# jac99/Egonn

Measured on AMD Instinct MI355X. Metric: LiDAR scans/sec (descriptor extraction), 50k-pt clouds @ 0.1m voxel, higher is better.
Workload: dtype f32

## Files before the change

egonn_amd/_lib.py:

```python
from __future__ import annotations

import ctypes as C
import os
from typing import List, Optional, Sequence

import numpy as np
import torch

_HERE = os.path.dirname(os.path.abspath(__file__))
LIB_PATH = os.path.join(_HERE, "lib", "libegonn_hip.so")

QUANT_CARTESIAN, QUANT_POLAR = 0, 1
FLAG_DISABLE_GLOBAL, FLAG_DISABLE_LOCAL, FLAG_IGNORE_KP_REGRESSOR, FLAG_BF16 = 1, 2, 4, 8
FLAG_POOL_SPOC, FLAG_POOL_MAC = 16, 32
MINKFPN_SPLIT_TOPDOWN = 1
MINKFPN_BLOCKS = {'BasicBlock': 0, 'ECABasicBlock': 1}
MINKFPN_POOLING = {None: 0, 'GeM': 1, 'MAC': 2, 'SPoC': 3}

_P = C.c_void_p
_SIGS = [
    ("egonn_ctx_create", C.c_int, [C.POINTER(_P), C.c_int, C.c_int]),
    ("egonn_ctx_destroy", None, [_P]),
    ("egonn_last_error", C.c_char_p, []),
    ("egonn_debug_set_naive_conv", C.c_int, [_P, C.c_int]),
    ("egonn_debug_set_ksplit", C.c_int, [_P, C.c_int, C.c_int, C.c_int, C.c_int, C.c_int]),
    ("egonn_debug_set_resident", C.c_int, [_P, C.c_int, C.c_int]),
    ("egonn_debug_keep_level_features", C.c_int, [_P, C.c_int]),
    ("egonn_debug_set_trace", C.c_int, [_P]),
    ("egonn_prepare_maps", C.c_int, [_P, C.c_int, _P]),
    ("egonn_debug_rowgroup_tables", C.c_int, [_P, C.c_int, C.c_int, _P, _P, C.c_int64, C.POINTER(C.c_int64), _P]),
    ("egonn_debug_rowgroup_perm", C.c_int, [_P, C.c_int, C.c_int, _P, C.c_int64, C.POINTER(C.c_int64), _P]),
    ("egonn_debug_radix_sort_scratch_bytes", C.c_int64, [C.c_int64, C.c_int]),
    ("egonn_debug_radix_sort", C.c_int, [_P, _P, _P, _P, C.c_int64, C.c_int, _P, _P, C.c_int, C.c_int, C.c_int,
                                         C.POINTER(C.c_int32), _P, C.c_int64, _P]),
    ("egonn_debug_dense_group3", C.c_int, [_P, _P, _P, _P, _P, _P, _P]),
    ("egonn_debug_global_tail_scratch_bytes", C.c_int64, [C.c_int64]),
    ("egonn_debug_global_tail", C.c_int, [_P, _P, C.c_int, C.c_int64, _P, _P, _P, _P, _P, _P, C.c_int, C.c_int, _P, _P, _P, C.c_int64, _P]),
    ("egonn_voxelize", C.c_int, [_P, _P, C.POINTER(C.c_int64), C.c_int, C.c_int, C.POINTER(C.c_float), _P]),
    ("egonn_ctx_reserve", C.c_int, [_P, C.c_int64, C.c_int, C.POINTER(C.c_int64)]),
    ("egonn_voxelize_device", C.c_int, [_P, _P, C.c_int64, _P, C.c_int, C.c_int, C.POINTER(C.c_float), _P]),
    ("egonn_plan_status", C.c_int, [_P, _P]),
    ("egonn_ctx_set_exact_fp32", C.c_int, [_P, C.c_int]),
    ("egonn_ctx_set_operand_autoscale", C.c_int, [_P, C.c_int]),
    ("egonn_level_capacity", C.c_int, [_P, C.c_int, C.POINTER(C.c_int64)]),
    ("egonn_graph_begin", C.c_int, [_P]),
    ("egonn_graph_end", C.c_int, [_P, C.POINTER(_P)]),
# ... 277 lines not shown
                       "gx", "gy", "gz", "block", "lds", "kparts")


def debug_sconv_choice(kind: int, level: int, cin: int, cout: int, cap_groups: int, *, code: int = 0, bf16: int = 0, gated: int = 0,
                       split_io: int = 0, residual: int = 0, split_max_level: int = 5, autoscale: int = 0, resident_mask: int = -1,
                       max_workgroups: int = 0, kparts: int = -1, kw: int = -1, col_parts: int = -1) -> dict:
    arg = (C.c_int32 * 16)(int(code), kind, level, cin, cout, int(bf16), int(gated), split_io, int(residual), split_max_level,
                           int(autoscale), resident_mask, max_workgroups, kparts, kw, col_parts)
    out = (C.c_int32 * 20)()
    check(load().egonn_debug_sconv_choice(arg, int(cap_groups), out))
    d = dict(zip(SCONV_CHOICE_FIELDS, out))
    d["route"], d["kernel"] = SCONV_ROUTES[d["route"]], SCONV_ROUTES[d["kernel"]]
    return d


DENSE_ROUTES = ("none", "stream", "lds", "small", "tile", "plain")


def debug_dense_route(rows: int, cin: int, cout: int, form: int = -1, gate_scans: int = 0):
    out = (C.c_int32 * 5)()
    check(load().egonn_debug_dense_route(int(rows), int(cin), int(cout), int(form), int(gate_scans), out))
    return (DENSE_ROUTES[out[0]],) + tuple(out[1:])


def debug_radix_sort(keys_in, vals_in, keys_out, vals_out, n: int, nbits: int, n_dev=None, seg_offsets=None, idx_bits: int = 0,
                     either_pair: bool = False, scratch_buf=None, scratch_bytes: Optional[int] = None) -> int:
    lib = load()
    B = 0 if seg_offsets is None else seg_offsets.numel() - 1
    need = lib.egonn_debug_radix_sort_scratch_bytes(int(n), B)
    if scratch_buf is None:
# ... 180 lines not shown
        ng, _ = self.map_groups(map_kind, level_out)
        K = 27 if map_kind == 0 else 8
        gm = torch.empty(ng, dtype=torch.int32, device=self.device)
        sn = torch.empty((ng, K, 16), dtype=torch.int32, device=self.device) if with_rows else None
        n = C.c_int64()
        self._call(self.lib.egonn_debug_rowgroup_tables, self.h, map_kind, level_out, gm.data_ptr(),
                   sn.data_ptr() if with_rows else None, ng, C.byref(n))
        return gm, sn

    def rowgroup_perm(self, map_kind: int, level_out: int):
        ng, _ = self.map_groups(map_kind, level_out)
        pm = torch.empty((ng, 16), dtype=torch.int32, device=self.device)
        n = C.c_int64()
        self._call(self.lib.egonn_debug_rowgroup_perm, self.h, map_kind, level_out, pm.data_ptr(), ng, C.byref(n))
        return pm

    def set_naive_conv(self, on):
        check(self.lib.egonn_debug_set_naive_conv(self.h, int(on)))

    def keep_level_features(self, on: bool):
        check(self.lib.egonn_debug_keep_level_features(self.h, int(bool(on))))

    def set_exact_fp32(self, on: bool):
        check(self.lib.egonn_ctx_set_exact_fp32(self.h, int(bool(on))))

    def set_operand_autoscale(self, on: bool):
        check(self.lib.egonn_ctx_set_operand_autoscale(self.h, int(bool(on))))

    def set_ksplit(self, map_class: int, level: int, kparts: int = -1, kw: int = -1, col_parts: int = -1):
        check(self.lib.egonn_debug_set_ksplit(self.h, int(map_class), int(level), int(kparts), int(kw), int(col_parts)))
# ... 390 lines not shown
```

egonn_amd/csrc/common.h:

```cpp
#pragma once
#include <hip/hip_runtime.h>
#include <atomic>
#include <stdint.h>
#include <stdio.h>
#include <string.h>
#include <string>
#include <vector>

#define EGONN_MAX_LEVELS 10
#define EGONN_NUM_LEVELS 8
#define EGONN_MAX_BATCH 4096

#define API extern "C" __attribute__((visibility("default")))

namespace egonn {

void set_error(const char* fmt, ...);
#define EGONN_OK 0
#define EGONN_ERR_INVALID 1
#define EGONN_ERR_HIP 2
#define EGONN_ERR_RANGE 3
#define EGONN_ERR_STATE 4
#define EGONN_ERR_CAPACITY 5
#define EGONN_ERR_FP16_RANGE 6
// ... 139 lines not shown
struct Plan {
  bool valid = false;
  bool built_reserved = false;
  bool exact = false;
  int64_t cap_points = 0;
  int64_t* scan_off = nullptr;
  int batch = 0;
  int coord_bits = 16;
  int64_t n_input = 0;
  Level lv[EGONN_MAX_LEVELS];
  int64_t cap[EGONN_MAX_LEVELS] = {};
  int32_t* perm0 = nullptr;
  int32_t* g0 = nullptr;
  uint64_t* t2m = nullptr;
  int32_t* t2s = nullptr;
  std::vector<int32_t> boff_host[EGONN_NUM_LEVELS];
};

enum ProfKind { PK_CONV0 = 0, PK_K3 = 1, PK_K2S2 = 2, PK_TCONV = 3, PK_OTHER = 4 };
struct ProfRec {
  char name[64];
  int kind, level, K, cin, cout;
  int es;
  hipEvent_t e0, e1;
};
struct Profiler {
  int mode = 0;
  char filter[64] = "";
  std::vector<ProfRec> recs;
  std::vector<ProfRec> graph_recs;
// ... 4 lines not shown
struct Switches {
  bool debug_sync;
  bool no_presplit;
  bool no_fused_down;
  bool no_fused_lateral;
  bool no_gated_k2s2;
  bool no_fused_ghead;
  bool no_fused_gtail;
  bool no_packed_laterals;
  bool no_split_heads;
  bool no_tail_split;
  bool no_task_order;
  bool flat_sort, sort_pairs;
  bool no_search67;
  bool no_dense_stream;
  int split_max_level;
  int split_max_level_k8;
  int split_cfg;
  int rg_first_pass;
  const char* ksplit[5];
};
const Switches& switches();

struct KsRule {
  int8_t kparts[2][EGONN_NUM_LEVELS];
  int8_t kw[2][EGONN_NUM_LEVELS];
  int8_t col_parts[EGONN_NUM_LEVELS];
};

static constexpr int SCONV_RESIDENT_DEFAULT = 6;
// ... 104 lines not shown
```

egonn_amd/csrc/conv.hip:

```cpp
#include <algorithm>
#include <type_traits>
#include <utility>

#include "common.h"
#include <hip/hip_ext.h>
#include "kernels.h"
#include "rowmath.h"

namespace egonn {

__global__ void sconv_naive_kernel(const float* __restrict__ in, const int32_t* __restrict__ nbr,
                                   const float* __restrict__ W, const float* __restrict__ scale,
                                   const float* __restrict__ shift, int relu, float* __restrict__ out, int32_t n_out,
                                   int K, int cin, int cout) {
  const int64_t t = (int64_t)blockIdx.x * blockDim.x + threadIdx.x;
  if (t >= (int64_t)n_out * cout) return;
  const int32_t o = (int32_t)(t / cout);
  const int co = (int)(t - (int64_t)o * cout);
  float acc = 0.f;
  for (int k = 0; k < K; ++k) {
    const int32_t j = nbr[(int64_t)o * K + k];
    if (j < 0) continue;
    const float* f = in + (int64_t)j * cin;
    const float* w = W + ((int64_t)k * cin) * cout + co;
// ... 156 lines not shown
          }
          *reinterpret_cast<uint2*>(reinterpret_cast<uint16_t*>(out_v) + (int64_t)orow * COUT0 + nt * 16 + 4 * g4) =
              make_uint2(w[0] | (w[1] << 16), w[2] | (w[3] << 16));
        } else {
          *reinterpret_cast<f32x4*>(reinterpret_cast<float*>(out_v) + (int64_t)orow * COUT0 + nt * 16 + 4 * g4) = o;
        }
      }
    }
    __builtin_amdgcn_wave_barrier();
    g_cur = g_nxt; lk_cur = lk_nxt;
    g_nxt = g_nn; lk_nxt = lk_nn;
  }
}

typedef short bf16x8_c0 __attribute__((ext_vector_type(8)));
template <bool OUT_BF16>
__global__ __launch_bounds__(256) void conv0_k5_unit_kernel(const uint64_t* __restrict__ vkeys,
                                                             const int32_t* __restrict__ g0,
                                                             const uint64_t* __restrict__ t2m,
                                                             const int32_t* __restrict__ counts, int32_t cap2, int32_t cap0,
                                                             const float* __restrict__ W,
                                                             const float* __restrict__ scale, const float* __restrict__ shift,
                                                             int relu, void* __restrict__ out_v,
                                                             const uint16_t* __restrict__ lut,
                                                             const uint4* __restrict__ wpk) {
  constexpr int MS = 29;
  constexpr int LUT_STRIDE = 136;
  __shared__ uint64_t s_m[4][16][MS];
  __shared__ __attribute__((aligned(16))) uint16_t s_lut[64 * LUT_STRIDE];
  const int tid = threadIdx.x, lane = tid & 63, wave = tid >> 6;
  const int l15 = lane & 15, g4 = lane >> 4;
  const int32_t nvox = min(__builtin_amdgcn_readfirstlane(counts[0]), cap0);
  const int32_t n2 = min(__builtin_amdgcn_readfirstlane(counts[2]), cap2);
  const int32_t ntiles = (nvox + 15) >> 4;
  for (int e = tid; e < 64 * 128 / 2; e += 256) {
    const int r = e >> 6, c = e & 63;
    reinterpret_cast<uint32_t*>(s_lut)[r * (LUT_STRIDE / 2) + c] = reinterpret_cast<const uint32_t*>(lut)[e];
  }
  if (tid < 64) s_m[tid >> 4][tid & 15][27] = 0ull;
  bf16x8_c0 wf[2][4][3];
  if (wpk) {
#pragma unroll
    for (int nt = 0; nt < 2; ++nt)
#pragma unroll
      for (int j = 0; j < 4; ++j)
#pragma unroll
        for (int sp = 0; sp < 3; ++sp) wf[nt][j][sp] = __builtin_bit_cast(bf16x8_c0, wpk[((nt * 4 + j) * 3 + sp) * 64 + lane]);
  } else
#pragma unroll
  for (int nt = 0; nt < 2; ++nt)
#pragma unroll
    for (int j = 0; j < 4; ++j) {
      uint32_t h[3][8];
#pragma unroll
      for (int e = 0; e < 8; ++e) {
        const int k = 32 * j + 8 * g4 + e;
        float w = (k < 125) ? W[k * COUT0 + nt * 16 + l15] : 0.f;
#pragma unroll
        for (int sp = 0; sp < 3; ++sp) {
          const uint32_t b = f2bf_rn(w);
          h[sp][e] = b;
          w -= __uint_as_float(b << 16);
        }
      }
#pragma unroll
      for (int sp = 0; sp < 3; ++sp) {
        const uint4 pk = make_uint4(h[sp][0] | (h[sp][1] << 16), h[sp][2] | (h[sp][3] << 16), h[sp][4] | (h[sp][5] << 16),
                                    h[sp][6] | (h[sp][7] << 16));
        wf[nt][j][sp] = __builtin_bit_cast(bf16x8_c0, pk);
      }
    }
  f32x4 sc[2], sh[2];
#pragma unroll
  for (int nt = 0; nt < 2; ++nt) {
    sc[nt] = scale ? *reinterpret_cast<const f32x4*>(scale + nt * 16 + 4 * g4) : (f32x4){1.f, 1.f, 1.f, 1.f};
    sh[nt] = scale ? *reinterpret_cast<const f32x4*>(shift + nt * 16 + 4 * g4) : (f32x4){0.f, 0.f, 0.f, 0.f};
  }
  __syncthreads();
  const __amdgpu_buffer_rsrc_t m_rsrc =
      __builtin_amdgcn_make_buffer_rsrc(const_cast<uint64_t*>(t2m), 0, (int)((uint32_t)n2 * 27u * 8u), 0x00020000);
  const __amdgpu_buffer_rsrc_t g_rsrc =
      __builtin_amdgcn_make_buffer_rsrc(const_cast<int32_t*>(g0), 0, (int)((uint32_t)nvox * 4u), 0x00020000);
  const __amdgpu_buffer_rsrc_t k_rsrc =
      __builtin_amdgcn_make_buffer_rsrc(const_cast<uint64_t*>(vkeys), 0, (int)((uint32_t)nvox * 8u), 0x00020000);
  const int tstep = gridDim.x * 4;
  constexpr int NE = (16 * 27 + 63) / 64;
// ... 44 lines not shown
      uint32_t pk[4];
#pragma unroll
      for (int q = 0; q < 4; ++q) {
        const uint32_t e0 = ew[q] & 0xFFFFu, e1 = ew[q] >> 16;
        const uint64_t m0 = *reinterpret_cast<const uint64_t*>(mrow + (e0 >> 6));
        const uint64_t m1 = *reinterpret_cast<const uint64_t*>(mrow + (e1 >> 6));
        const uint32_t h0 = (uint32_t)(m0 >> (e0 & 63)) & 1u, h1 = (uint32_t)(m1 >> (e1 & 63)) & 1u;
        pk[q] = h0 * 0x3F80u + h1 * 0x3F800000u;
      }
      const bf16x8_c0 av = __builtin_bit_cast(bf16x8_c0, make_uint4(pk[0], pk[1], pk[2], pk[3]));
#pragma unroll
      for (int sp = 0; sp < 3; ++sp)
#pragma unroll
        for (int nt = 0; nt < 2; ++nt) acc[nt] = __builtin_amdgcn_mfma_f32_16x16x32_bf16(wf[nt][j][sp], av, acc[nt], 0, 0, 0);
    }
    const int32_t orow = r0 + l15;
    if (orow < nvox) {
#pragma unroll
      for (int nt = 0; nt < 2; ++nt) {
        f32x4 o = acc[nt] * sc[nt] + sh[nt];
        if (relu) {
#pragma unroll
          for (int u = 0; u < 4; ++u) o[u] = fmaxf(o[u], 0.f);
        }
        if constexpr (OUT_BF16) {
          *reinterpret_cast<uint2*>(reinterpret_cast<uint16_t*>(out_v) + (int64_t)orow * COUT0 + nt * 16 + 4 * g4) =
              make_uint2(f2bf_rn(o[0]) | (f2bf_rn(o[1]) << 16), f2bf_rn(o[2]) | (f2bf_rn(o[3]) << 16));
        } else {
          *reinterpret_cast<f32x4*>(reinterpret_cast<float*>(out_v) + (int64_t)orow * COUT0 + nt * 16 + 4 * g4) = o;
        }
      }
    }
    __builtin_amdgcn_wave_barrier();
    g_cur = g_nxt; lk_cur = lk_nxt;
    g_nxt = g_nn; lk_nxt = lk_nn;
  }
}

__global__ void conv0_pack_unit_kernel(const float* __restrict__ W, uint4* __restrict__ wpk) {
  const int t = blockIdx.x * blockDim.x + threadIdx.x;
  if (t >= 2 * 4 * 64) return;
  const int lane = t & 63, j = (t >> 6) & 3, nt = t >> 8;
  const int l15 = lane & 15, g4 = lane >> 4;
  uint32_t h[3][8];
#pragma unroll
  for (int e = 0; e < 8; ++e) {
    const int k = 32 * j + 8 * g4 + e;
// ... 48 lines not shown
  EGONN_TRY(conv0_lut_init(ctx));
  EGONN_REQUIRE(cout == COUT0, EGONN_ERR_INVALID, "conv0: %d output channels not supported (expected %d)", cout, COUT0);
  const Level& V = P.lv[0];
  const Level& B = P.lv[2];
  if (P.cap[0] == 0) return EGONN_OK;
  const int32_t ntiles = (int32_t)cdiv(P.cap[0], 16);
  const unsigned grid = (unsigned)std::min<int64_t>(cdiv(ntiles, 4), 512);
  EGONN_REQUIRE(P.g0 && P.t2m && P.t2s, EGONN_ERR_STATE, "conv0: plan has no block-neighbourhood table");
#define EGONN_CONV0_LAUNCH(U, OB)                                                                                      \
  hipLaunchKernelGGL((conv0_k5_kernel<U, OB>), dim3(grid), dim3(256), 0, stream, feat, V.keys, P.g0, P.t2m, P.t2s,       \
                     ctx->dev_counts, (int32_t)P.cap[2], (int32_t)P.cap[0], W, scale, shift, relu, out, ctx->conv0_lut)
  if (feat) {
    if (out_bf16) EGONN_CONV0_LAUNCH(false, true); else EGONN_CONV0_LAUNCH(false, false);
  } else if (ctx->sconv.set.family == SCONV_PLAIN) {
    if (out_bf16) EGONN_CONV0_LAUNCH(true, true); else EGONN_CONV0_LAUNCH(true, false);
  } else {
    if (out_bf16)
      hipLaunchKernelGGL((conv0_k5_unit_kernel<true>), dim3(grid), dim3(256), 0, stream, V.keys, P.g0, P.t2m, ctx->dev_counts,
                         (int32_t)P.cap[2], (int32_t)P.cap[0], W, scale, shift, relu, out, ctx->conv0_lut,
                         reinterpret_cast<const uint4*>(wpk));
    else
      hipLaunchKernelGGL((conv0_k5_unit_kernel<false>), dim3(grid), dim3(256), 0, stream, V.keys, P.g0, P.t2m, ctx->dev_counts,
                         (int32_t)P.cap[2], (int32_t)P.cap[0], W, scale, shift, relu, out, ctx->conv0_lut,
                         reinterpret_cast<const uint4*>(wpk));
  }
#undef EGONN_CONV0_LAUNCH
  HIP_CHECK(hipGetLastError());
  return EGONN_OK;
}

}
```

egonn_amd/csrc/coords.hip:

```cpp
#include "common.h"

#include <algorithm>
#include <stdarg.h>

namespace egonn {

static thread_local char g_err[1024] = "";
void set_error(const char* fmt, ...) {
  va_list ap;
  va_start(ap, fmt);
  vsnprintf(g_err, sizeof(g_err), fmt, ap);
  va_end(ap);
}
const char* last_error() { return g_err; }

const Switches& switches() {
  static const Switches sw = [] {
    auto on = [](const char* name) { return getenv(name) != nullptr; };
    auto num = [](const char* name, int unset) { const char* e = getenv(name); return e ? atoi(e) : unset; };
    const char* ds = getenv("EGONN_DEBUG_SYNC");
    return Switches{.debug_sync = ds && ds[0] == '1', .no_presplit = on("EGONN_NO_PRESPLIT"), .no_fused_down = on("EGONN_NO_FUSED_DOWN"),
                    .no_fused_lateral = on("EGONN_NO_FUSED_LATERAL"), .no_gated_k2s2 = on("EGONN_NO_GATED_K2S2"),
                    .no_fused_ghead = on("EGONN_NO_FUSED_GHEAD"), .no_fused_gtail = on("EGONN_NO_FUSED_GTAIL"),
                    .no_packed_laterals = on("EGONN_NO_PACKED_LATERALS"), .no_split_heads = on("EGONN_NO_SPLIT_HEADS"),
                    .no_tail_split = on("EGONN_NO_TAIL_SPLIT"), .no_task_order = on("EGONN_NO_TASK_ORDER"),
                    .flat_sort = on("EGONN_FLAT_SORT"), .sort_pairs = on("EGONN_SORT_PAIRS"), .no_search67 = on("EGONN_NO_SEARCH67"),
                    .no_dense_stream = on("EGONN_NO_DENSE_STREAM"),
                    .split_max_level = num("EGONN_SPLIT_MAX_LEVEL", -1), .split_max_level_k8 = num("EGONN_SPLIT_MAX_LEVEL_K8", -1),
                    .split_cfg = num("EGONN_SPLIT_CFG", 0), .rg_first_pass = num("EGONN_RG_FIRST_PASS", 0),
                    .ksplit = {getenv("EGONN_KSPLIT"), getenv("EGONN_KSPLIT8"), getenv("EGONN_KSPLIT_KW"), getenv("EGONN_KSPLIT_KW8"),
                               getenv("EGONN_KSPLIT_PARTS")}};
  }();
  return sw;
}

hipEvent_t Profiler::get() {
  if (!pool.empty()) {
    hipEvent_t e = pool.back();
    pool.pop_back();
    return e;
  }
  hipEvent_t e = nullptr;
// ... 322 lines not shown
  const int32_t e = cs2[cs1[j + 1]];
  const uint64_t* k = a.keys[L - 2];
  uint64_t m = 0;
  for (int32_t r = s; r < e; ++r) m |= 1ull << (k[r] & 63);
  a.mask[L][j] = m;
  a.bstart[L][j] = s;
}

__device__ static inline int32_t find_key(const uint64_t* __restrict__ keys, int32_t n, uint64_t q) {
  int32_t lo = 0, hi = n;
  while (lo < hi) {
    const int32_t mid = (lo + hi) >> 1;
    if (keys[mid] < q) lo = mid + 1; else hi = mid;
  }
  return (lo < n && keys[lo] == q) ? lo : -1;
}

__device__ static inline uint32_t bit_of_local(uint32_t lx, uint32_t ly, uint32_t lz) {
  return (lx & 1) | ((ly & 1) << 1) | ((lz & 1) << 2) | ((lx & 2) << 2) | ((ly & 2) << 3) | ((lz & 2) << 4);
}

__device__ static inline int32_t lookup_local(const uint64_t* nbm, const int32_t* nbs, int32_t nx, int32_t ny,
                                              int32_t nz) {
  const int32_t sx = (nx < 0) ? 0 : (nx > 3 ? 2 : 1);
  const int32_t sy = (ny < 0) ? 0 : (ny > 3 ? 2 : 1);
  const int32_t sz = (nz < 0) ? 0 : (nz > 3 ? 2 : 1);
  const int32_t slot = sx + 3 * sy + 9 * sz;
  const uint32_t bit = bit_of_local((uint32_t)nx & 3, (uint32_t)ny & 3, (uint32_t)nz & 3);
  const uint64_t m = nbm[slot];
  if (!((m >> bit) & 1)) return -1;
  return nbs[slot] + __popcll(m & ((1ull << bit) - 1));
}

struct Adj27Args {
// ... 37 lines not shown
struct Nbr27Job {
  const uint64_t* vkeys;
  const int32_t* badj;
  const uint64_t* bmask;
  const int32_t* bstart;
  int32_t* nbr;
  int32_t level, cap_blocks, cap_vox;
};
struct Blk27Args {
  const int32_t* badj;
  const uint64_t* bmask;
  const int32_t* bstart;
  int32_t cap2;
  uint64_t* t2m;
  int32_t* t2s;
};
struct Nbr27Pair {
  Nbr27Job job[2];
  const int32_t* counts;
  uint32_t split;
  uint32_t tail_at;
  Blk27Args blk;
};
__device__ static inline void blk27_body(const Blk27Args& b, const int32_t* __restrict__ counts, uint32_t vblock) {
  const int32_t t = (int32_t)(vblock * 256 + threadIdx.x);
  if (t >= level_rows(counts, 2, b.cap2) * 27) return;
  const int32_t a = b.badj[t];
  b.t2m[t] = a >= 0 ? b.bmask[a] : 0ull;
  b.t2s[t] = a >= 0 ? b.bstart[a] : 0;
}
__global__ __launch_bounds__(256) void nbr27_kernel(const Nbr27Pair a) {
  if (blockIdx.x >= a.tail_at) {
    blk27_body(a.blk, a.counts, blockIdx.x - a.tail_at);
    return;
  }
  const bool second = blockIdx.x >= a.split;
  const Nbr27Job& J = a.job[second ? 1 : 0];
  const uint64_t* __restrict__ vkeys = J.vkeys;
  const int32_t* __restrict__ badj = J.badj;
  const uint64_t* __restrict__ bmask = J.bmask;
  const int32_t* __restrict__ bstart = J.bstart;
  const int32_t* __restrict__ counts = a.counts;
  int32_t* __restrict__ nbr = J.nbr;
  const int level = J.level;
// ... 343 lines not shown
  const int search_from = (search67_ok && P.cap[NL - 4] <= 8192 && P.cap[NL - 3] <= 8192) ? NL - 4 : NL - 2;
  ta.b_adj2 = 0;
  ta.adj2 = ta.adj;
  if (search_from == NL - 4) {
    Level& V = P.lv[NL - 4];
    Level& V1 = P.lv[NL - 3];
    const int32_t nv = (int32_t)P.cap[NL - 4], nv1 = (int32_t)P.cap[NL - 3];
    ta.adj2 = Adj27Args{V.keys, V1.keys, counts, NL - 4, NL - 3, cb - (NL - 4), cb - (NL - 3), nv, nv1, V.nbr27, V1.nbr27};
    ta.b_adj2 = (unsigned)cdiv(((int64_t)nv + nv1) * 27, 256);
  }
  const int32_t n0 = (int32_t)P.cap[0], n2 = (int32_t)P.cap[2];
  {
    P.g0 = A.alloc<int32_t>(n0);
    P.t2m = A.alloc<uint64_t>((size_t)n2 * 27);
    P.t2s = A.alloc<int32_t>((size_t)n2 * 27);
    EGONN_REQUIRE(P.g0 && P.t2m && P.t2s, EGONN_ERR_STATE, "plan arena too small");
    ta.parent0 = P.lv[0].parent; ta.parent1 = P.lv[1].parent; ta.g0 = P.g0; ta.cap0 = n0;
    ta.b_gp = (unsigned)cdiv(n0, 256);
  }
  {
    Nbr8TArgs& na = ta.na;
    na.prefix[0] = na.prefix[1] = 0;
    na.counts = counts;
    for (int l = 1; l < EGONN_NUM_LEVELS; ++l) {
      Level& V = P.lv[l];
      const int32_t nv = (int32_t)P.cap[l];
      V.nbr8 = A.alloc<int32_t>((size_t)nv * 8);
      V.nbrT = A.alloc<int32_t>((size_t)nv * 8);
      EGONN_REQUIRE(V.nbr8 && V.nbrT, EGONN_ERR_STATE, "plan arena too small");
      na.cstart[l] = V.cstart;
      na.ckeys[l] = P.lv[l - 1].keys;
// ... 5 lines not shown
    }
    na.cstart[0] = nullptr; na.ckeys[0] = nullptr; na.parent[0] = nullptr; na.keys[0] = nullptr;
    na.nbr8[0] = nullptr; na.nbrT[0] = nullptr;
    ta.b_n8 = (unsigned)cdiv(na.prefix[EGONN_NUM_LEVELS], 256);
  }
  {
    const unsigned nb = ta.b_mask + ta.b_adj + ta.b_adj2 + ta.b_gp + ta.b_n8;
    if (nb > 0) hipLaunchKernelGGL(plan_tables_kernel, dim3(nb), dim3(256), 0, stream, ta);
  }

  Nbr27Pair pair;
  int npair = 0;
  pair.counts = counts;
  pair.split = 0;
  pair.tail_at = ~0u;
  pair.blk = Blk27Args{nullptr, nullptr, nullptr, 0, nullptr, nullptr};
  bool blk_done = false;
  auto flush = [&](bool last) {
    if (npair == 0 && !(last && !blk_done && n0 > 0)) return;
    if (npair == 1) pair.job[1] = pair.job[0];
    const unsigned g0 = npair >= 1 ? pair.split : 0u, g1 = npair == 2 ? (unsigned)cdiv(pair.job[1].cap_blocks, 4) : 0u;
    if (npair == 0) { pair.split = 0; pair.job[0] = Nbr27Job{nullptr, nullptr, nullptr, nullptr, nullptr, 1, 0, 0}; pair.job[1] = pair.job[0]; }
    unsigned extra = 0;
    pair.tail_at = ~0u;
    if (last && !blk_done && n0 > 0) {
      pair.tail_at = g0 + g1;
      pair.blk = Blk27Args{P.lv[2].nbr27, P.lv[2].mask, P.lv[2].bstart, n2, P.t2m, P.t2s};
      extra = (unsigned)cdiv((int64_t)n2 * 27, 256);
      blk_done = true;
    }
    if (g0 + g1 + extra > 0) hipLaunchKernelGGL(nbr27_kernel, dim3(g0 + g1 + extra), dim3(256), 0, stream, pair);
    npair = 0;
  };
  for (int l = search_from - 1; l >= 1; --l) {
    Level& V = P.lv[l];
    const int32_t nv = (int32_t)P.cap[l];
    if (nv == 0) continue;
    const Level& Bk = P.lv[l + 2];
    if (npair == 1 && pair.job[0].level != l + 1) flush(false);
    Nbr27Job& J = pair.job[npair];
    J.vkeys = V.keys; J.badj = Bk.nbr27; J.bmask = Bk.mask; J.bstart = Bk.bstart; J.nbr = V.nbr27;
    J.level = l; J.cap_blocks = (int32_t)P.cap[l + 2]; J.cap_vox = nv;
    if (npair == 0) pair.split = (unsigned)cdiv(P.cap[l + 2], 4);
// ... 55 lines not shown
    EGONN_REQUIRE(nj < RG_MAX_JOBS, EGONN_ERR_INVALID, "rowgroups: too many maps in one request");
    jobs[nj].rg = &rg;
    jobs[nj].nbr = nbr;
    jobs[nj].n_dev = ctx->dev_counts + l;
    jobs[nj].boff = V.boff;
    jobs[nj].cap_rows = (int32_t)P.cap[l];
    ++nj;
  }
  if (nj == 0) return EGONN_OK;
  EGONN_TRY(rowgroup_build(jobs, nj, P.batch, stream));
  for (int j = 0; j < nj; ++j) jobs[j].rg->built = true;
  return EGONN_OK;
}

static size_t plan_arena_bytes(int64_t n, int B) {
  size_t per_row = 2 * (8 + 4) + NL * (8 + 4 + 4 + 8 + 4) + 4 + 9 * 27 * 4 + 7 * (8 + 8) * 4 + 4 + 27 * 12 + 8 * 4;
  per_row += 2 * ((27 + 1) * 4 + 2 + 2 * ((8 + 1) * 4 + 2));
  const size_t rg_round = (size_t)(B + 8) * 1024 * (28 + 14 + 2 * 9) * 4 * EGONN_NUM_LEVELS;
  return (size_t)(n + 8) * per_row + (size_t)(B + 1) * 4 * EGONN_NUM_LEVELS + (size_t)cdiv(n, PYR_TILE) * NL * 4 + rg_round +
         (1 << 20);
}

int plan_from_points(Ctx* ctx, const float* points, const int64_t* scan_offsets, int64_t n_cap, int offsets_on_device,
                     int B, int mode, const float* step, hipStream_t stream) {
  ctx->plan.valid = false;
  EGONN_REQUIRE(B >= 1 && B <= EGONN_MAX_BATCH, EGONN_ERR_INVALID, "batch size %d outside [1,%d]", B, EGONN_MAX_BATCH);
  EGONN_REQUIRE(mode == 0 || mode == 1, EGONN_ERR_INVALID, "unknown quantiser mode %d", mode);
  int64_t n;
  if (!offsets_on_device) {
    n = scan_offsets[B];
    EGONN_REQUIRE(scan_offsets[0] == 0 && n >= 1, EGONN_ERR_INVALID, "empty input (n=%lld points)", (long long)n);
// ... 76 lines not shown
}

int plan_level_coords(Ctx* ctx, int level, int32_t* out, hipStream_t stream) {
  EGONN_REQUIRE(ctx->plan.valid, EGONN_ERR_STATE, "no coordinate plan (call egonn_voxelize / egonn_coords_set first)");
  EGONN_REQUIRE(level >= 0 && level < EGONN_MAX_LEVELS, EGONN_ERR_INVALID, "level %d out of range", level);
  EGONN_TRY(plan_sync(ctx, stream));
  const Level& L = ctx->plan.lv[level];
  if (L.n == 0) return EGONN_OK;
  hipLaunchKernelGGL(decode_coords_kernel, dim3((unsigned)cdiv(L.n, 256)), dim3(256), 0, stream, L.keys, (int32_t)L.n,
                     level, ctx->plan.coord_bits, out);
  HIP_CHECK(hipGetLastError());
  return EGONN_OK;
}

}
```

include/egonn_hip.h:

```cpp
#ifndef EGONN_HIP_H
#define EGONN_HIP_H

#include <stdint.h>

#ifdef __cplusplus
extern "C" {
#endif

typedef struct egonn_ctx egonn_ctx;
typedef struct egonn_model egonn_model;

enum { EGONN_QUANT_CARTESIAN = 0, EGONN_QUANT_POLAR = 1 };
enum { EGONN_STATUS_OK = 0, EGONN_STATUS_INVALID = 1, EGONN_STATUS_HIP = 2, EGONN_STATUS_RANGE = 3, EGONN_STATUS_STATE = 4,
       EGONN_STATUS_CAPACITY = 5,
       EGONN_STATUS_FP16_RANGE = 6 };
enum { EGONN_FLAG_DISABLE_GLOBAL = 1, EGONN_FLAG_DISABLE_LOCAL = 2, EGONN_FLAG_IGNORE_KP_REGRESSOR = 4,
       EGONN_FLAG_BF16 = 8,
       EGONN_FLAG_POOL_SPOC = 16, EGONN_FLAG_POOL_MAC = 32 };

int egonn_ctx_create(egonn_ctx** ctx, int device, int coord_bits);
void egonn_ctx_destroy(egonn_ctx* ctx);
const char* egonn_last_error(void);
int egonn_debug_set_naive_conv(egonn_ctx* ctx, int on);
int egonn_debug_set_ksplit(egonn_ctx* ctx, int map_class, int level, int kparts, int kw, int col_parts);
int egonn_debug_set_resident(egonn_ctx* ctx, int mask, int max_workgroups);
int egonn_debug_keep_level_features(egonn_ctx* ctx, int on);
int egonn_debug_set_trace(void* device_buffer);
int egonn_debug_rowgroup_tables(egonn_ctx* ctx, int map_kind, int level_out, uint32_t* gmask_out, int32_t* snbr_out,
                                int64_t capacity_groups, int64_t* n_groups, void* stream);
int egonn_debug_rowgroup_perm(egonn_ctx* ctx, int map_kind, int level_out, int32_t* perm_out, int64_t capacity_groups,
                              int64_t* n_groups, void* stream);
int64_t egonn_debug_radix_sort_scratch_bytes(int64_t n, int n_segments);
int egonn_debug_radix_sort(uint64_t* keys_in, uint32_t* vals_in, uint64_t* keys_out, uint32_t* vals_out, int64_t n, int nbits,
                           const int64_t* n_dev, const int64_t* seg_offsets, int n_segments, int idx_bits, int either_pair,
                           int32_t* result_pair, void* scratch, int64_t scratch_bytes, void* stream);
int egonn_debug_dense_group3(const float* const in[3], const int64_t rows_capacity[3], const int32_t* const n_dev[3],
                             const float* const weight[3], const float* const packed[3], float* const out[3], void* stream);
int64_t egonn_debug_global_tail_scratch_bytes(int64_t rows_capacity);
int egonn_debug_global_tail(const float* g5, const int32_t* row_offsets, int batch_size, int64_t rows_capacity, const int32_t* n_dev,
                            const float* w0, const float* b0, const float* w1, const float* b1, const float* p, int pooling, int form,
                            float* partial, float* out, void* scratch, int64_t scratch_bytes, void* stream);

int egonn_voxelize(egonn_ctx* ctx, const float* points, const int64_t* scan_offsets, int batch_size, int quant_mode,
                   const float* step, void* stream);
int egonn_ctx_reserve(egonn_ctx* ctx, int64_t max_points, int batch_size, const int64_t* level_capacity);
int egonn_voxelize_device(egonn_ctx* ctx, const float* points, int64_t n_rows, const int64_t* scan_offsets_dev,
// ... 359 lines not shown
```

Measured before the change: 23390.

## Precompute per-block 8x8x8 halo occupancy cubes for conv0 unit kernel

The level-2 neighbour table build now also emits a 64-byte occupancy cube for each level-2 block, covering its 8x8x8 halo. The default conv0 unit kernel reads this cube with buffer loads and extracts the 5x5x5 neighbourhood bits with shifts, so it no longer gathers 27 masks into LDS and goes through the LUT. This aims to cut per-tile LDS staging and LUT lookups in conv0, and it prefetches the next tile's cube. The cost is an extra 64 bytes per level-2 row in the plan arena and more work in the blk27 kernel. The old LUT path stays behind an environment switch.

```diff
diff --git a/egonn_amd/_lib.py b/egonn_amd/_lib.py
--- a/egonn_amd/_lib.py
+++ b/egonn_amd/_lib.py
@@ -30,6 +30,8 @@
     ("egonn_prepare_maps", C.c_int, [_P, C.c_int, _P]),
     ("egonn_debug_rowgroup_tables", C.c_int, [_P, C.c_int, C.c_int, _P, _P, C.c_int64, C.POINTER(C.c_int64), _P]),
     ("egonn_debug_rowgroup_perm", C.c_int, [_P, C.c_int, C.c_int, _P, C.c_int64, C.POINTER(C.c_int64), _P]),
+    ("egonn_debug_conv0_cubes", C.c_int, [_P, _P, C.c_int64, C.POINTER(C.c_int64), C.c_int, _P]),
+    ("egonn_debug_conv0_cube_host", C.c_int, [_P, C.c_int64, _P, _P]),
     ("egonn_debug_radix_sort_scratch_bytes", C.c_int64, [C.c_int64, C.c_int]),
     ("egonn_debug_radix_sort", C.c_int, [_P, _P, _P, _P, C.c_int64, C.c_int, _P, _P, C.c_int, C.c_int, C.c_int,
                                          C.POINTER(C.c_int32), _P, C.c_int64, _P]),
@@ -337,6 +339,15 @@
     return d
 
 
+def debug_conv0_cube_host(masks):
+    import numpy as np
+    m = np.ascontiguousarray(masks, dtype=np.uint64).reshape(-1, 27)
+    cubes = np.zeros((m.shape[0], 64), np.uint8)
+    ops = np.zeros((m.shape[0], 64, 4), np.uint32)
+    check(load().egonn_debug_conv0_cube_host(m.ctypes.data, m.shape[0], cubes.ctypes.data, ops.ctypes.data))
+    return cubes, ops
+
+
 DENSE_ROUTES = ("none", "stream", "lds", "small", "tile", "plain")
 
 
@@ -547,6 +558,14 @@
         n = C.c_int64()
         self._call(self.lib.egonn_debug_rowgroup_perm, self.h, map_kind, level_out, pm.data_ptr(), ng, C.byref(n))
         return pm
+
+    def conv0_cubes(self, poison: bool = False):
+        cap = self.level_capacity(2)
+        out = torch.empty(cap * 64 + 64, dtype=torch.uint8, device=self.device)
+        n = C.c_int64()
+        self._call(self.lib.egonn_debug_conv0_cubes, self.h, out.data_ptr(), out.numel(), C.byref(n), int(bool(poison)))
+        assert n.value == cap
+        return out, cap
 
     def set_naive_conv(self, on):
         check(self.lib.egonn_debug_set_naive_conv(self.h, int(on)))
diff --git a/egonn_amd/csrc/common.h b/egonn_amd/csrc/common.h
--- a/egonn_amd/csrc/common.h
+++ b/egonn_amd/csrc/common.h
@@ -177,6 +177,7 @@
   int32_t* g0 = nullptr;
   uint64_t* t2m = nullptr;
   int32_t* t2s = nullptr;
+  unsigned char* cube = nullptr;
   std::vector<int32_t> boff_host[EGONN_NUM_LEVELS];
 };
 
@@ -211,6 +212,7 @@
   bool flat_sort, sort_pairs;
   bool no_search67;
   bool no_dense_stream;
+  bool no_conv0_cube;
   int split_max_level;
   int split_max_level_k8;
   int split_cfg;
diff --git a/egonn_amd/csrc/conv.hip b/egonn_amd/csrc/conv.hip
--- a/egonn_amd/csrc/conv.hip
+++ b/egonn_amd/csrc/conv.hip
@@ -3,6 +3,7 @@
 #include <utility>
 
 #include "common.h"
+#include "conv0_cube.h"
 #include <hip/hip_ext.h>
 #include "kernels.h"
 #include "rowmath.h"
@@ -194,16 +195,72 @@
 }
 
 typedef short bf16x8_c0 __attribute__((ext_vector_type(8)));
+
+__device__ __forceinline__ void conv0_unit_wfrag(bf16x8_c0 (&wf)[2][4][3], const float* __restrict__ W,
+                                                 const uint4* __restrict__ wpk, int lane) {
+  const int l15 = lane & 15, g4 = lane >> 4;
+  if (wpk) {
+#pragma unroll
+    for (int nt = 0; nt < 2; ++nt)
+#pragma unroll
+      for (int j = 0; j < 4; ++j)
+#pragma unroll
+        for (int sp = 0; sp < 3; ++sp) wf[nt][j][sp] = __builtin_bit_cast(bf16x8_c0, wpk[((nt * 4 + j) * 3 + sp) * 64 + lane]);
+  } else
+#pragma unroll
+  for (int nt = 0; nt < 2; ++nt)
+#pragma unroll
+    for (int j = 0; j < 4; ++j) {
+      uint32_t h[3][8];
+#pragma unroll
+      for (int e = 0; e < 8; ++e) {
+        const int k = 32 * j + 8 * g4 + e;
+        float w = (k < 125) ? W[k * COUT0 + nt * 16 + l15] : 0.f;
+#pragma unroll
+        for (int sp = 0; sp < 3; ++sp) {
+          const uint32_t b = f2bf_rn(w);
+          h[sp][e] = b;
+          w -= __uint_as_float(b << 16);
+        }
+      }
+#pragma unroll
+      for (int sp = 0; sp < 3; ++sp) {
+        const uint4 pk = make_uint4(h[sp][0] | (h[sp][1] << 16), h[sp][2] | (h[sp][3] << 16), h[sp][4] | (h[sp][5] << 16),
+                                    h[sp][6] | (h[sp][7] << 16));
+        wf[nt][j][sp] = __builtin_bit_cast(bf16x8_c0, pk);
+      }
+    }
+}
+
 template <bool OUT_BF16>
-__global__ __launch_bounds__(256) void conv0_k5_unit_kernel(const uint64_t* __restrict__ vkeys,
-                                                             const int32_t* __restrict__ g0,
-                                                             const uint64_t* __restrict__ t2m,
-                                                             const int32_t* __restrict__ counts, int32_t cap2, int32_t cap0,
-                                                             const float* __restrict__ W,
-                                                             const float* __restrict__ scale, const float* __restrict__ shift,
-                                                             int relu, void* __restrict__ out_v,
-                                                             const uint16_t* __restrict__ lut,
-                                                             const uint4* __restrict__ wpk) {
+__device__ __forceinline__ void conv0_unit_store(const f32x4 (&acc)[2], const f32x4 (&sc)[2], const f32x4 (&sh)[2], int relu,
+                                                 void* __restrict__ out_v, int32_t orow, int g4) {
+#pragma unroll
+  for (int nt = 0; nt < 2; ++nt) {
+    f32x4 o = acc[nt] * sc[nt] + sh[nt];
+    if (relu) {
+#pragma unroll
+      for (int u = 0; u < 4; ++u) o[u] = fmaxf(o[u], 0.f);
+    }
+    if constexpr (OUT_BF16) {
+      *reinterpret_cast<uint2*>(reinterpret_cast<uint16_t*>(out_v) + (int64_t)orow * COUT0 + nt * 16 + 4 * g4) =
+          make_uint2(f2bf_rn(o[0]) | (f2bf_rn(o[1]) << 16), f2bf_rn(o[2]) | (f2bf_rn(o[3]) << 16));
+    } else {
+      *reinterpret_cast<f32x4*>(reinterpret_cast<float*>(out_v) + (int64_t)orow * COUT0 + nt * 16 + 4 * g4) = o;
+    }
+  }
+}
+
+template <bool OUT_BF16>
+__global__ __launch_bounds__(256) void conv0_k5_unit_lut_kernel(const uint64_t* __restrict__ vkeys,
+                                                                 const int32_t* __restrict__ g0,
+                                                                 const uint64_t* __restrict__ t2m,
+                                                                 const int32_t* __restrict__ counts, int32_t cap2, int32_t cap0,
+                                                                 const float* __restrict__ W,
+                                                                 const float* __restrict__ scale, const float* __restrict__ shift,
+                                                                 int relu, void* __restrict__ out_v,
+                                                                 const uint16_t* __restrict__ lut,
+                                                                 const uint4* __restrict__ wpk) {
   constexpr int MS = 29;
   constexpr int LUT_STRIDE = 136;
   __shared__ uint64_t s_m[4][16][MS];
@@ -219,37 +276,7 @@
   }
   if (tid < 64) s_m[tid >> 4][tid & 15][27] = 0ull;
   bf16x8_c0 wf[2][4][3];
-  if (wpk) {
-#pragma unroll
-    for (int nt = 0; nt < 2; ++nt)
-#pragma unroll
-      for (int j = 0; j < 4; ++j)
-#pragma unroll
-        for (int sp = 0; sp < 3; ++sp) wf[nt][j][sp] = __builtin_bit_cast(bf16x8_c0, wpk[((nt * 4 + j) * 3 + sp) * 64 + lane]);
-  } else
-#pragma unroll
-  for (int nt = 0; nt < 2; ++nt)
-#pragma unroll
-    for (int j = 0; j < 4; ++j) {
-      uint32_t h[3][8];
-#pragma unroll
-      for (int e = 0; e < 8; ++e) {
-        const int k = 32 * j + 8 * g4 + e;
-        float w = (k < 125) ? W[k * COUT0 + nt * 16 + l15] : 0.f;
-#pragma unroll
-        for (int sp = 0; sp < 3; ++sp) {
-          const uint32_t b = f2bf_rn(w);
-          h[sp][e] = b;
-          w -= __uint_as_float(b << 16);
-        }
-      }
-#pragma unroll
-      for (int sp = 0; sp < 3; ++sp) {
-        const uint4 pk = make_uint4(h[sp][0] | (h[sp][1] << 16), h[sp][2] | (h[sp][3] << 16), h[sp][4] | (h[sp][5] << 16),
-                                    h[sp][6] | (h[sp][7] << 16));
-        wf[nt][j][sp] = __builtin_bit_cast(bf16x8_c0, pk);
-      }
-    }
+  conv0_unit_wfrag(wf, W, wpk, lane);
   f32x4 sc[2], sh[2];
 #pragma unroll
   for (int nt = 0; nt < 2; ++nt) {
@@ -324,23 +351,89 @@
 #pragma unroll
         for (int nt = 0; nt < 2; ++nt) acc[nt] = __builtin_amdgcn_mfma_f32_16x16x32_bf16(wf[nt][j][sp], av, acc[nt], 0, 0, 0);
     }
-    const int32_t orow = r0 + l15;
-    if (orow < nvox) {
-#pragma unroll
-      for (int nt = 0; nt < 2; ++nt) {
-        f32x4 o = acc[nt] * sc[nt] + sh[nt];
-        if (relu) {
-#pragma unroll
-          for (int u = 0; u < 4; ++u) o[u] = fmaxf(o[u], 0.f);
-        }
-        if constexpr (OUT_BF16) {
-          *reinterpret_cast<uint2*>(reinterpret_cast<uint16_t*>(out_v) + (int64_t)orow * COUT0 + nt * 16 + 4 * g4) =
-              make_uint2(f2bf_rn(o[0]) | (f2bf_rn(o[1]) << 16), f2bf_rn(o[2]) | (f2bf_rn(o[3]) << 16));
-        } else {
-          *reinterpret_cast<f32x4*>(reinterpret_cast<float*>(out_v) + (int64_t)orow * COUT0 + nt * 16 + 4 * g4) = o;
-        }
-      }
-    }
+    if (r0 + l15 < nvox) conv0_unit_store<OUT_BF16>(acc, sc, sh, relu, out_v, r0 + l15, g4);
+    __builtin_amdgcn_wave_barrier();
+    g_cur = g_nxt; lk_cur = lk_nxt;
+    g_nxt = g_nn; lk_nxt = lk_nn;
+  }
+}
+
+template <bool OUT_BF16>
+__global__ __launch_bounds__(256) void conv0_k5_unit_kernel(const uint64_t* __restrict__ vkeys,
+                                                             const int32_t* __restrict__ g0,
+                                                             const unsigned char* __restrict__ cube,
+                                                             const int32_t* __restrict__ counts, int32_t cap2, int32_t cap0,
+                                                             const float* __restrict__ W,
+                                                             const float* __restrict__ scale, const float* __restrict__ shift,
+                                                             int relu, void* __restrict__ out_v,
+                                                             const uint4* __restrict__ wpk) {
+  constexpr int CS = 56;
+  __shared__ __attribute__((aligned(8))) unsigned char s_c[4][16 * CS];
+  const int tid = threadIdx.x, lane = tid & 63, wave = tid >> 6;
+  const int l15 = lane & 15, g4 = lane >> 4;
+  const int32_t nvox = min(__builtin_amdgcn_readfirstlane(counts[0]), cap0);
+  const int32_t n2 = min(__builtin_amdgcn_readfirstlane(counts[2]), cap2);
+  const int32_t ntiles = (nvox + 15) >> 4;
+  bf16x8_c0 wf[2][4][3];
+  conv0_unit_wfrag(wf, W, wpk, lane);
+  f32x4 sc[2], sh[2];
+#pragma unroll
+  for (int nt = 0; nt < 2; ++nt) {
+    sc[nt] = scale ? *reinterpret_cast<const f32x4*>(scale + nt * 16 + 4 * g4) : (f32x4){1.f, 1.f, 1.f, 1.f};
+    sh[nt] = scale ? *reinterpret_cast<const f32x4*>(shift + nt * 16 + 4 * g4) : (f32x4){0.f, 0.f, 0.f, 0.f};
+  }
+  const __amdgpu_buffer_rsrc_t c_rsrc =
+      __builtin_amdgcn_make_buffer_rsrc(const_cast<unsigned char*>(cube), 0, (int)((uint32_t)n2 * 64u + 16u), 0x00020000);
+  const __amdgpu_buffer_rsrc_t g_rsrc =
+      __builtin_amdgcn_make_buffer_rsrc(const_cast<int32_t*>(g0), 0, (int)((uint32_t)nvox * 4u), 0x00020000);
+  const __amdgpu_buffer_rsrc_t k_rsrc =
+      __builtin_amdgcn_make_buffer_rsrc(const_cast<uint64_t*>(vkeys), 0, (int)((uint32_t)nvox * 8u), 0x00020000);
+  const int tstep = gridDim.x * 4;
+  auto row_info = [&](int32_t tile, int32_t& g, uint32_t& lkbits) {
+    const uint32_t r = (uint32_t)tile * 16u + (uint32_t)l15;
+    g = __builtin_amdgcn_raw_buffer_load_b32(g_rsrc, (int)(r * 4u), 0, 0);
+    lkbits = (uint32_t)__builtin_amdgcn_raw_buffer_load_b32(k_rsrc, (int)(r * 8u), 0, 0) & 63u;
+  };
+  typedef uint32_t u32x4_c0 __attribute__((ext_vector_type(4)));
+  auto cube_issue = [&](int32_t g, uint32_t lk) -> u32x4_c0 {
+    const uint32_t lz = ((lk >> 2) & 1u) | ((lk >> 4) & 2u);
+    const uint32_t off = g4 < 3 ? (uint32_t)g * 64u + 8u * lz + 16u * (uint32_t)g4 : 0xFFFFFFF0u;
+    return __builtin_amdgcn_raw_buffer_load_b128(c_rsrc, (int)off, 0, 0);
+  };
+  int32_t tile = blockIdx.x * 4 + wave;
+  int32_t g_cur, g_nxt, g_nn;
+  uint32_t lk_cur, lk_nxt, lk_nn;
+  row_info(tile, g_cur, lk_cur);
+  row_info(tile + tstep, g_nxt, lk_nxt);
+  u32x4_c0 pc = cube_issue(g_cur, lk_cur);
+  unsigned char* img = &s_c[wave][l15 * CS];
+  for (; tile < ntiles; tile += tstep) {
+    const int32_t r0 = tile * 16;
+    if (g4 < 3) {
+      *reinterpret_cast<uint2*>(img + 16 * g4) = make_uint2(pc[0], pc[1]);
+      *reinterpret_cast<uint2*>(img + 16 * g4 + 8) = make_uint2(pc[2], pc[3]);
+    }
+    __builtin_amdgcn_fence(__ATOMIC_ACQ_REL, "wavefront");
+    __builtin_amdgcn_wave_barrier();
+    pc = cube_issue(g_nxt, lk_nxt);
+    row_info(tile + 2 * tstep, g_nn, lk_nn);
+    uint32_t lx, ly, lz, f[5], N[4];
+    conv0_local(lk_cur, lx, ly, lz);
+#pragma unroll
+    for (int d = 0; d < 5; ++d) f[d] = conv0_plane_field(*reinterpret_cast<const uint64_t*>(img + 8 * d), 8 * ly + lx);
+    conv0_pack_fields(f, N);
+    f32x4 acc[2] = {{0.f, 0.f, 0.f, 0.f}, {0.f, 0.f, 0.f, 0.f}};
+#pragma unroll
+    for (int j = 0; j < 4; ++j) {
+      const uint32_t byte = (N[j] >> (8 * g4)) & 0xFFu;
+      const bf16x8_c0 av = __builtin_bit_cast(bf16x8_c0, make_uint4(conv0_bf16_pair(byte, 0), conv0_bf16_pair(byte, 1),
+                                                                    conv0_bf16_pair(byte, 2), conv0_bf16_pair(byte, 3)));
+#pragma unroll
+      for (int sp = 0; sp < 3; ++sp)
+#pragma unroll
+        for (int nt = 0; nt < 2; ++nt) acc[nt] = __builtin_amdgcn_mfma_f32_16x16x32_bf16(wf[nt][j][sp], av, acc[nt], 0, 0, 0);
+    }
+    if (r0 + l15 < nvox) conv0_unit_store<OUT_BF16>(acc, sc, sh, relu, out_v, r0 + l15, g4);
     __builtin_amdgcn_wave_barrier();
     g_cur = g_nxt; lk_cur = lk_nxt;
     g_nxt = g_nn; lk_nxt = lk_nn;
@@ -419,15 +512,23 @@
     if (out_bf16) EGONN_CONV0_LAUNCH(false, true); else EGONN_CONV0_LAUNCH(false, false);
   } else if (ctx->sconv.set.family == SCONV_PLAIN) {
     if (out_bf16) EGONN_CONV0_LAUNCH(true, true); else EGONN_CONV0_LAUNCH(true, false);
-  } else {
+  } else if (switches().no_conv0_cube) {
     if (out_bf16)
-      hipLaunchKernelGGL((conv0_k5_unit_kernel<true>), dim3(grid), dim3(256), 0, stream, V.keys, P.g0, P.t2m, ctx->dev_counts,
+      hipLaunchKernelGGL((conv0_k5_unit_lut_kernel<true>), dim3(grid), dim3(256), 0, stream, V.keys, P.g0, P.t2m, ctx->dev_counts,
                          (int32_t)P.cap[2], (int32_t)P.cap[0], W, scale, shift, relu, out, ctx->conv0_lut,
                          reinterpret_cast<const uint4*>(wpk));
     else
-      hipLaunchKernelGGL((conv0_k5_unit_kernel<false>), dim3(grid), dim3(256), 0, stream, V.keys, P.g0, P.t2m, ctx->dev_counts,
+      hipLaunchKernelGGL((conv0_k5_unit_lut_kernel<false>), dim3(grid), dim3(256), 0, stream, V.keys, P.g0, P.t2m, ctx->dev_counts,
                          (int32_t)P.cap[2], (int32_t)P.cap[0], W, scale, shift, relu, out, ctx->conv0_lut,
                          reinterpret_cast<const uint4*>(wpk));
+  } else {
+    EGONN_REQUIRE(P.cube, EGONN_ERR_STATE, "conv0: plan has no halo-cube table");
+    if (out_bf16)
+      hipLaunchKernelGGL((conv0_k5_unit_kernel<true>), dim3(grid), dim3(256), 0, stream, V.keys, P.g0, P.cube, ctx->dev_counts,
+                         (int32_t)P.cap[2], (int32_t)P.cap[0], W, scale, shift, relu, out, reinterpret_cast<const uint4*>(wpk));
+    else
+      hipLaunchKernelGGL((conv0_k5_unit_kernel<false>), dim3(grid), dim3(256), 0, stream, V.keys, P.g0, P.cube, ctx->dev_counts,
+                         (int32_t)P.cap[2], (int32_t)P.cap[0], W, scale, shift, relu, out, reinterpret_cast<const uint4*>(wpk));
   }
 #undef EGONN_CONV0_LAUNCH
   HIP_CHECK(hipGetLastError());
diff --git a/egonn_amd/csrc/conv0_cube.h b/egonn_amd/csrc/conv0_cube.h
--- /dev/null
+++ b/egonn_amd/csrc/conv0_cube.h
@@ -0,0 +1,53 @@
+#pragma once
+#include <stdint.h>
+
+namespace egonn {
+
+__host__ __device__ static inline uint32_t bit_of_local(uint32_t lx, uint32_t ly, uint32_t lz) {
+  return (lx & 1) | ((ly & 1) << 1) | ((lz & 1) << 2) | ((lx & 2) << 2) | ((ly & 2) << 3) | ((lz & 2) << 4);
+}
+
+__host__ __device__ static inline uint32_t conv0_xrow(uint64_t m, uint32_t ly, uint32_t lz) {
+  const uint32_t base = bit_of_local(0, ly, lz);
+  return (uint32_t)((m >> base) & 3u) | ((uint32_t)((m >> (base + 8)) & 3u) << 2);
+}
+
+__host__ __device__ static inline uint32_t conv0_cube_row(const uint64_t* m27, uint32_t yp, uint32_t zp) {
+  const uint32_t sy = yp < 2 ? 0u : (yp < 6 ? 1u : 2u), sz = zp < 2 ? 0u : (zp < 6 ? 1u : 2u);
+  const uint32_t ly = (yp - 2u) & 3u, lz = (zp - 2u) & 3u;
+  const uint64_t* m = m27 + 3 * sy + 9 * sz;
+  return (conv0_xrow(m[0], ly, lz) >> 2) | (conv0_xrow(m[1], ly, lz) << 2) | ((conv0_xrow(m[2], ly, lz) & 3u) << 6);
+}
+
+__host__ __device__ static inline void conv0_local(uint32_t lk, uint32_t& lx, uint32_t& ly, uint32_t& lz) {
+  lx = (lk & 1) | ((lk >> 2) & 2);
+  ly = ((lk >> 1) & 1) | ((lk >> 3) & 2);
+  lz = ((lk >> 2) & 1) | ((lk >> 4) & 2);
+}
+
+__host__ __device__ static inline uint32_t conv0_plane_field(uint64_t P, uint32_t sh) {
+  const uint64_t t = (P >> sh) & 0x1F1F1F1F1Full;
+  const uint32_t lo = (uint32_t)t, hi = (uint32_t)(t >> 32);
+  return (lo & 0x1Fu) | ((lo >> 3) & 0x3E0u) | ((lo >> 6) & 0x7C00u) | ((lo >> 9) & 0xF8000u) | (hi << 20);
+}
+
+__host__ __device__ static inline void conv0_pack_fields(const uint32_t f[5], uint32_t N[4]) {
+  N[0] = f[0] | (f[1] << 25);
+  N[1] = (f[1] >> 7) | (f[2] << 18);
+  N[2] = (f[2] >> 14) | (f[3] << 11);
+  N[3] = (f[3] >> 21) | (f[4] << 4);
+}
+
+__host__ __device__ static inline void conv0_operand(const uint64_t cube64[8], uint32_t lk, uint32_t N[4]) {
+  uint32_t lx, ly, lz, f[5];
+  conv0_local(lk, lx, ly, lz);
+  for (int d = 0; d < 5; ++d) f[d] = conv0_plane_field(cube64[lz + d], 8 * ly + lx);
+  conv0_pack_fields(f, N);
+}
+
+__host__ __device__ static inline uint32_t conv0_bf16_pair(uint32_t byte, int q) {
+  const uint32_t x = (byte >> (2 * q)) & 3u;
+  return ((x * 0x8001u) & 0x10001u) * 0x3F80u;
+}
+
+}
diff --git a/egonn_amd/csrc/coords.hip b/egonn_amd/csrc/coords.hip
--- a/egonn_amd/csrc/coords.hip
+++ b/egonn_amd/csrc/coords.hip
@@ -1,4 +1,6 @@
 #include "common.h"
+#include "conv0_cube.h"
+#include "model.h"
 
 #include <algorithm>
 #include <stdarg.h>
@@ -25,7 +27,7 @@
                     .no_packed_laterals = on("EGONN_NO_PACKED_LATERALS"), .no_split_heads = on("EGONN_NO_SPLIT_HEADS"),
                     .no_tail_split = on("EGONN_NO_TAIL_SPLIT"), .no_task_order = on("EGONN_NO_TASK_ORDER"),
                     .flat_sort = on("EGONN_FLAT_SORT"), .sort_pairs = on("EGONN_SORT_PAIRS"), .no_search67 = on("EGONN_NO_SEARCH67"),
-                    .no_dense_stream = on("EGONN_NO_DENSE_STREAM"),
+                    .no_dense_stream = on("EGONN_NO_DENSE_STREAM"), .no_conv0_cube = on("EGONN_NO_CONV0_CUBE"),
                     .split_max_level = num("EGONN_SPLIT_MAX_LEVEL", -1), .split_max_level_k8 = num("EGONN_SPLIT_MAX_LEVEL_K8", -1),
                     .split_cfg = num("EGONN_SPLIT_CFG", 0), .rg_first_pass = num("EGONN_RG_FIRST_PASS", 0),
                     .ksplit = {getenv("EGONN_KSPLIT"), getenv("EGONN_KSPLIT8"), getenv("EGONN_KSPLIT_KW"), getenv("EGONN_KSPLIT_KW8"),
@@ -378,10 +380,6 @@
     if (keys[mid] < q) lo = mid + 1; else hi = mid;
   }
   return (lo < n && keys[lo] == q) ? lo : -1;
-}
-
-__device__ static inline uint32_t bit_of_local(uint32_t lx, uint32_t ly, uint32_t lz) {
-  return (lx & 1) | ((ly & 1) << 1) | ((lz & 1) << 2) | ((lx & 2) << 2) | ((ly & 2) << 3) | ((lz & 2) << 4);
 }
 
 __device__ static inline int32_t lookup_local(const uint64_t* nbm, const int32_t* nbs, int32_t nx, int32_t ny,
@@ -449,6 +447,7 @@
   int32_t cap2;
   uint64_t* t2m;
   int32_t* t2s;
+  unsigned char* cube;
 };
 struct Nbr27Pair {
   Nbr27Job job[2];
@@ -458,11 +457,35 @@
   Blk27Args blk;
 };
 __device__ static inline void blk27_body(const Blk27Args& b, const int32_t* __restrict__ counts, uint32_t vblock) {
-  const int32_t t = (int32_t)(vblock * 256 + threadIdx.x);
-  if (t >= level_rows(counts, 2, b.cap2) * 27) return;
-  const int32_t a = b.badj[t];
-  b.t2m[t] = a >= 0 ? b.bmask[a] : 0ull;
-  b.t2s[t] = a >= 0 ? b.bstart[a] : 0;
+  __shared__ uint64_t s_m27[4][4 * 27];
+  const int lane = threadIdx.x & 63, wave = threadIdx.x >> 6;
+  const int32_t n2 = level_rows(counts, 2, b.cap2);
+  const int32_t j0 = (int32_t)(vblock * 16 + wave * 4);
+  if (j0 >= n2) return;
+#pragma unroll
+  for (int e = 0; e < 2; ++e) {
+    const int t = lane + 64 * e;
+    if (t < 4 * 27) {
+      const int64_t ent = (int64_t)j0 * 27 + t;
+      uint64_t m = 0ull;
+      if (ent < (int64_t)n2 * 27) {
+        const int32_t a = b.badj[ent];
+        m = a >= 0 ? b.bmask[a] : 0ull;
+        b.t2m[ent] = m;
+        b.t2s[ent] = a >= 0 ? b.bstart[a] : 0;
+      }
+      s_m27[wave][t] = m;
+    }
+  }
+  __builtin_amdgcn_fence(__ATOMIC_ACQ_REL, "wavefront");
+  __builtin_amdgcn_wave_barrier();
+  const int q = lane >> 4, h = lane & 15;
+  if (j0 + q >= n2) return;
+  const uint64_t* m27 = s_m27[wave] + 27 * q;
+  uint32_t w = 0;
+#pragma unroll
+  for (uint32_t r = 0; r < 4; ++r) w |= conv0_cube_row(m27, 4u * ((uint32_t)h & 1u) + r, (uint32_t)h >> 1) << (8 * r);
+  reinterpret_cast<uint32_t*>(b.cube)[(int64_t)(j0 + q) * 16 + h] = w;
 }
 __global__ __launch_bounds__(256) void nbr27_kernel(const Nbr27Pair a) {
   if (blockIdx.x >= a.tail_at) {
@@ -836,7 +859,8 @@
     P.g0 = A.alloc<int32_t>(n0);
     P.t2m = A.alloc<uint64_t>((size_t)n2 * 27);
     P.t2s = A.alloc<int32_t>((size_t)n2 * 27);
-    EGONN_REQUIRE(P.g0 && P.t2m && P.t2s, EGONN_ERR_STATE, "plan arena too small");
+    P.cube = A.alloc<unsigned char>((size_t)n2 * 64 + 64);
+    EGONN_REQUIRE(P.g0 && P.t2m && P.t2s && P.cube, EGONN_ERR_STATE, "plan arena too small");
     ta.parent0 = P.lv[0].parent; ta.parent1 = P.lv[1].parent; ta.g0 = P.g0; ta.cap0 = n0;
     ta.b_gp = (unsigned)cdiv(n0, 256);
   }
@@ -872,7 +896,7 @@
   pair.counts = counts;
   pair.split = 0;
   pair.tail_at = ~0u;
-  pair.blk = Blk27Args{nullptr, nullptr, nullptr, 0, nullptr, nullptr};
+  pair.blk = Blk27Args{nullptr, nullptr, nullptr, 0, nullptr, nullptr, nullptr};
   bool blk_done = false;
   auto flush = [&](bool last) {
     if (npair == 0 && !(last && !blk_done && n0 > 0)) return;
@@ -883,8 +907,8 @@
     pair.tail_at = ~0u;
     if (last && !blk_done && n0 > 0) {
       pair.tail_at = g0 + g1;
-      pair.blk = Blk27Args{P.lv[2].nbr27, P.lv[2].mask, P.lv[2].bstart, n2, P.t2m, P.t2s};
-      extra = (unsigned)cdiv((int64_t)n2 * 27, 256);
+      pair.blk = Blk27Args{P.lv[2].nbr27, P.lv[2].mask, P.lv[2].bstart, n2, P.t2m, P.t2s, P.cube};
+      extra = (unsigned)cdiv(n2, 16);
       blk_done = true;
     }
     if (g0 + g1 + extra > 0) hipLaunchKernelGGL(nbr27_kernel, dim3(g0 + g1 + extra), dim3(256), 0, stream, pair);
@@ -970,7 +994,7 @@
 }
 
 static size_t plan_arena_bytes(int64_t n, int B) {
-  size_t per_row = 2 * (8 + 4) + NL * (8 + 4 + 4 + 8 + 4) + 4 + 9 * 27 * 4 + 7 * (8 + 8) * 4 + 4 + 27 * 12 + 8 * 4;
+  size_t per_row = 2 * (8 + 4) + NL * (8 + 4 + 4 + 8 + 4) + 4 + 9 * 27 * 4 + 7 * (8 + 8) * 4 + 4 + 27 * 12 + 64 + 8 * 4;
   per_row += 2 * ((27 + 1) * 4 + 2 + 2 * ((8 + 1) * 4 + 2));
   const size_t rg_round = (size_t)(B + 8) * 1024 * (28 + 14 + 2 * 9) * 4 * EGONN_NUM_LEVELS;
   return (size_t)(n + 8) * per_row + (size_t)(B + 1) * 4 * EGONN_NUM_LEVELS + (size_t)cdiv(n, PYR_TILE) * NL * 4 + rg_round +
@@ -1077,3 +1101,29 @@
 }
 
 }
+
+using namespace egonn;
+
+API int egonn_debug_conv0_cubes(egonn_ctx* c, uint8_t* out, int64_t out_bytes, int64_t* cap_rows, int poison, void* stream) {
+  REQUIRE_PLAN(c);
+  HIP_CHECK(hipSetDevice(c->device));
+  const Plan& P = c->plan;
+  EGONN_REQUIRE(out && cap_rows && out_bytes >= 0 && P.cube, EGONN_ERR_INVALID, "debug_conv0_cubes: bad arguments");
+  const size_t bytes = (size_t)P.cap[2] * 64 + 64;
+  HIP_CHECK(hipMemcpyAsync(out, P.cube, std::min(bytes, (size_t)out_bytes), hipMemcpyDeviceToDevice, (hipStream_t)stream));
+  if (poison) HIP_CHECK(hipMemsetAsync(P.cube, 0xA5, bytes, (hipStream_t)stream));
+  *cap_rows = P.cap[2];
+  return EGONN_OK;
+}
+
+API int egonn_debug_conv0_cube_host(const uint64_t* masks, int64_t n_sets, uint8_t* cubes_out, uint32_t* operands_out) {
+  EGONN_REQUIRE(masks && cubes_out && n_sets >= 0, EGONN_ERR_INVALID, "debug_conv0_cube_host: bad arguments");
+  for (int64_t i = 0; i < n_sets; ++i) {
+    uint64_t planes[8];
+    for (uint32_t r = 0; r < 64; ++r) cubes_out[i * 64 + r] = (uint8_t)conv0_cube_row(masks + i * 27, r & 7u, r >> 3);
+    memcpy(planes, cubes_out + i * 64, 64);
+    if (operands_out)
+      for (uint32_t lk = 0; lk < 64; ++lk) conv0_operand(planes, lk, operands_out + (i * 64 + lk) * 4);
+  }
+  return EGONN_OK;
+}
diff --git a/include/egonn_hip.h b/include/egonn_hip.h
--- a/include/egonn_hip.h
+++ b/include/egonn_hip.h
@@ -30,6 +30,8 @@
                                 int64_t capacity_groups, int64_t* n_groups, void* stream);
 int egonn_debug_rowgroup_perm(egonn_ctx* ctx, int map_kind, int level_out, int32_t* perm_out, int64_t capacity_groups,
                               int64_t* n_groups, void* stream);
+int egonn_debug_conv0_cubes(egonn_ctx* ctx, uint8_t* out, int64_t out_bytes, int64_t* cap_rows, int poison, void* stream);
+int egonn_debug_conv0_cube_host(const uint64_t* masks, int64_t n_sets, uint8_t* cubes_out, uint32_t* operands_out);
 int64_t egonn_debug_radix_sort_scratch_bytes(int64_t n, int n_segments);
 int egonn_debug_radix_sort(uint64_t* keys_in, uint32_t* vals_in, uint64_t* keys_out, uint32_t* vals_out, int64_t n, int nbits,
                            const int64_t* n_dev, const int64_t* seg_offsets, int n_segments, int idx_bits, int either_pair,
```

Result: no change. 23540, median of 6 (+0.6%).
